# meuleman/epilogos

Hardware: AMD Instinct MI355X
Metric: Mbins scored/sec (S1, 18-state, 833 biosamples) (higher is better)
Workload: dtype u8

## Files before the change

### epilogos_amd/build.py

```python
import os
import shutil
import subprocess
from pathlib import Path

PKG = Path(__file__).resolve().parent
ROOT = PKG.parent
CSRC = PKG / "csrc"
LIB_DIR = PKG / "_lib"
LIB_PATH = LIB_DIR / "libepilogos_hip.so"
SOURCES = ["epg_abi.hip", "epg_s1.hip", "epg_s2.hip", "epg_s3.hip", "epg_s3_transpose.hip", "epg_s3_gemm.hip", "epg_s3_lanes.hip", "epg_null.hip", "epg_wide.hip", "epg_simsearch.hip",
           "epg_simsearch_prep.hip", "epg_scores_text.hip", "epg_groups.hip", "epg_null_exceed.hip", "epg_statebyline.hip", "epg_segments.hip", "epg_simsearch_pick.hip", "epg_census.hip", "epg_concordance.hip", "epg_gennorm.hip", "epg_pvals.hip", "epg_textout.hip", "epg_bgzf_inflate.hip", "epg_metrics_text.hip"]
PUBLIC_HEADERS = {"core": "epilogos_amd.h", "scores_text": "epilogos_scores_text.h", "groups": "epilogos_groups.h", "nulldraws": "epilogos_nulldraws.h",
                  "statebyline": "epilogos_statebyline.h", "segments": "epilogos_segments.h", "simsearch_pick": "epilogos_simsearch_pick.h",
                  "census": "epilogos_census.h", "concordance": "epilogos_concordance.h", "gennorm": "epilogos_gennorm.h"}
INTERNAL_HEADERS = {"pvals": "epg_pvals.h"}
WRITER_HEADERS = {"textout": "epg_textout.h"}
READER_HEADERS = {"bgzf_inflate": "epg_bgzf_inflate.h"}
METRICS_HEADERS = {"metrics_text": "epg_metrics_text.h"}
HEADERS = [CSRC / "epg_common.h", CSRC / "epg_count.h", CSRC / "epg_paircount.h", CSRC / "epg_parts.h", CSRC / "epg_pairdist.h", CSRC / "epg_text_scan.h", CSRC / "epg_text_rows.h", CSRC / "epg_fmt_f5.h", CSRC / "epg_fmt_e5.h", CSRC / "epg_bgzf_block.h", CSRC / "epg_bgzf_inflate_block.h",
           *[ROOT / "include" / name for name in PUBLIC_HEADERS.values()], *[CSRC / name for name in INTERNAL_HEADERS.values()], *[CSRC / name for name in WRITER_HEADERS.values()], *[CSRC / name for name in READER_HEADERS.values()], *[CSRC / name for name in METRICS_HEADERS.values()]]
ARCH = "gfx950"


def _hipcc():
    exe = shutil.which("hipcc") or "/opt/rocm/bin/hipcc"
    if not os.path.exists(exe):
        raise RuntimeError("hipcc not found: cannot build libepilogos_hip.so")
    return exe


def is_stale():
    if not LIB_PATH.exists():
        return True
    t = LIB_PATH.stat().st_mtime
    deps = [CSRC / s for s in SOURCES] + HEADERS
    return any(d.stat().st_mtime > t for d in deps)


IO_LIB_PATH = LIB_DIR / "libepilogos_io.so"
IO_SOURCE = CSRC / "epg_io.cpp"
IO_HEADER = ROOT / "include" / "epilogos_io.h"


def io_is_stale():
    if not IO_LIB_PATH.exists():
        return True
    t = IO_LIB_PATH.stat().st_mtime
    return any(f.stat().st_mtime > t for f in (IO_SOURCE, IO_HEADER, CSRC / "epg_deflate.h", CSRC / "epg_inflate.h", CSRC / "epg_crc32.h"))


def build_io_library(force=False, verbose=False):
    if not force and not io_is_stale():
        return IO_LIB_PATH
    LIB_DIR.mkdir(parents=True, exist_ok=True)
    cxx = shutil.which("g++") or shutil.which("c++")
    if cxx is None:
        raise RuntimeError("g++ not found: cannot build libepilogos_io.so")
    tmp = LIB_DIR / (IO_LIB_PATH.name + ".tmp.%d" % os.getpid())
    cmd = [cxx, "-O3", "-std=c++17", "-fPIC", "-shared", "-pthread", "-I" + str(ROOT / "include"), str(IO_SOURCE),
           "-lz", "-o", str(tmp)]
    if verbose:
        print(" ".join(cmd), flush=True)
    res = subprocess.run(cmd, capture_output=True, text=True)
    if res.returncode != 0:
        raise RuntimeError("g++ failed:\n" + res.stdout + res.stderr)
    os.replace(tmp, IO_LIB_PATH)
    return IO_LIB_PATH


OBJ_DIR = LIB_DIR / "obj"


def _compile_one(src, obj, extra_flags, verbose):
    cmd = [_hipcc(), "--offload-arch=" + ARCH, "-O3", "-std=c++17", "-fPIC", "-c",
           "-I" + str(ROOT / "include"), "-I" + str(CSRC), *extra_flags, str(src), "-o", str(obj)]
    if verbose:
        print(" ".join(cmd), flush=True)
    res = subprocess.run(cmd, capture_output=True, text=True)
    if res.returncode != 0:
        raise RuntimeError("hipcc failed on %s:\n%s%s" % (src.name, res.stdout, res.stderr))


def build_library(force=False, verbose=False, extra_flags=()):
    if os.environ.get("EPILOGOS_BUILD_EXPERIMENTS") == "1":
        extra_flags = tuple(extra_flags) + ("-DEPILOGOS_BUILD_EXPERIMENTS",)
    if not force and not is_stale():
        return LIB_PATH
    from concurrent.futures import ThreadPoolExecutor
    OBJ_DIR.mkdir(parents=True, exist_ok=True)
    flag_tag = OBJ_DIR / "flags.txt"
    flags_now = " ".join(extra_flags)
    same_flags = flag_tag.exists() and flag_tag.read_text() == flags_now
    hdr_t = max(h.stat().st_mtime for h in HEADERS)
    todo, objs = [], []
    for s in SOURCES:
        src, obj = CSRC / s, OBJ_DIR / (s + ".o")
        objs.append(obj)
        if force or not same_flags or not obj.exists() or obj.stat().st_mtime < max(src.stat().st_mtime, hdr_t):
            todo.append((src, obj))
    jobs = max(1, min(len(todo), int(os.environ.get("EPILOGOS_BUILD_JOBS", os.cpu_count() or 4))))
    if todo:
        with ThreadPoolExecutor(max_workers=jobs) as pool:
# ... 18 lines not shown
```

### epilogos_amd/csrc/epg_count.h

```cpp
#pragma once
#include "epg_common.h"
#include "epg_parts.h"

namespace epg {

#define EPG_B3(a, b, c, tt) ((u32)__builtin_amdgcn_bitop3_b32((int)(a), (int)(b), (int)(c), (tt)))

__device__ __forceinline__ u32 sel(u32 m, u32 x, u32 y) { return EPG_B3(m, x, y, 0xCA); }

__device__ __forceinline__ u32 dbl(u32 x) {
    u32 r;
    asm("v_add_u32 %0, %1, %1" : "=v"(r) : "v"(x));
    return r;
}

__device__ __forceinline__ void bit_planes(const u32 (&w)[8], u32 (&P)[5]) {
    const u32 n0 = sel(0x0f0f0f0fu, w[0], w[1] << 4);
    const u32 n1 = sel(0x0f0f0f0fu, w[2], w[3] << 4);
    const u32 n2 = sel(0x0f0f0f0fu, w[4], w[5] << 4);
    const u32 n3 = sel(0x0f0f0f0fu, w[6], w[7] << 4);
    const u32 m0 = sel(0x33333333u, n0, n1 << 2), m1 = sel(0x33333333u, n2, n3 << 2);
    const u32 r0 = sel(0xccccccccu, n1, n0 >> 2), r1 = sel(0xccccccccu, n3, n2 >> 2);
    P[0] = sel(0x55555555u, m0, dbl(m1)); P[1] = sel(0xaaaaaaaau, m1, m0 >> 1);
    P[2] = sel(0x55555555u, r0, dbl(r1)); P[3] = sel(0xaaaaaaaau, r1, r0 >> 1);
    const u32 c00 = sel(0x10101010u, w[0], dbl(w[4])), c01 = sel(0x10101010u, w[1], dbl(w[5]));
    const u32 c10 = sel(0x10101010u, w[2], dbl(w[6])), c11 = sel(0x10101010u, w[3], dbl(w[7]));
    const u32 d0 = sel(0x30303030u, c00, c10 << 2), d1 = sel(0x30303030u, c01, c11 << 2);
    P[4] = sel(0xf0f0f0f0u, d1, d0 >> 4);
}

__device__ __forceinline__ void low_three(const u32 (&P)[5], u32 (&L)[8]) {
    L[0] = EPG_B3(P[0], P[1], P[2], 0x01); L[1] = EPG_B3(P[0], P[1], P[2], 0x10); L[2] = EPG_B3(P[0], P[1], P[2], 0x04); L[3] = EPG_B3(P[0], P[1], P[2], 0x40);
    L[4] = EPG_B3(P[0], P[1], P[2], 0x02); L[5] = EPG_B3(P[0], P[1], P[2], 0x20); L[6] = EPG_B3(P[0], P[1], P[2], 0x08); L[7] = EPG_B3(P[0], P[1], P[2], 0x80);
}

__device__ __forceinline__ u32 indicator(const u32 (&L)[8], const u32 (&P)[5], int s) {
    switch (s >> 3) {
        case 0: return EPG_B3(L[s & 7], P[3], P[4], 0x10);
        case 1: return EPG_B3(L[s & 7], P[3], P[4], 0x40);
        case 2: return EPG_B3(L[s & 7], P[3], P[4], 0x20);
        default: return EPG_B3(L[s & 7], P[3], P[4], 0x80);
    }
}

template <int S>
__device__ __forceinline__ void count_group(const u32 (&w)[8], u32 (&cnt)[S]) {
    u32 P[5], L[8];
    bit_planes(w, P);
    low_three(P, L);
#pragma unroll
    for (int s = 0; s < S; ++s) cnt[s] += (u32)__builtin_popcount(indicator(L, P, s));
}

struct RowGeom {
    int chunks;
    int last;
    u32 tail[4];
};

__device__ __forceinline__ RowGeom make_geom(int N) {
    RowGeom g;
    g.chunks = (N + 15) >> 4;
    g.last = g.chunks - 1;
    const int t = N - 16 * g.last;
#pragma unroll
    for (int d = 0; d < 4; ++d) {
        int v = t - 4 * d;
        v = v < 0 ? 0 : (v > 4 ? 4 : v);
        g.tail[d] = v == 4 ? 0u : (0xffffffffu << (8 * v));
    }
    return g;
}

template <bool MAYBE_TAIL>
__device__ __forceinline__ void load_slot(const char* rowp, int i, int j, const RowGeom& g, u32* w) {
    const int c = 4 * i + j;
    if (!MAYBE_TAIL) {
        const uint4 v = ld16(rowp + 16 * c);
        w[0] = v.x; w[1] = v.y; w[2] = v.z; w[3] = v.w;
    } else {
        const int cc = c < g.last ? c : g.last;
        const uint4 v = ld16(rowp + 16 * cc);
        const u32 inv = c > g.last ? 0xffffffffu : 0u;
        const bool is_last = c == g.last;
// ... 20 lines not shown
}

template <int NC, typename Group>
__device__ __forceinline__ void for_each_group(const char* rowp, int j, const RowGeom& g, u32 (&cnt)[NC], Group group) {
    const int ngroups = (g.chunks + 7) >> 3;
    for (int t0 = 0; t0 < ngroups; t0 += 4) {
        u32 w[4][8];
#pragma unroll
        for (int k = 0; k < 4; ++k) {
            const int t = t0 + k;
            if (t < ngroups - 1) load_group<false>(rowp, t, j, g, w[k]);
            else if (t == ngroups - 1) load_group<true>(rowp, t, j, g, w[k]);
        }
#pragma unroll
        for (int k = 0; k < 4; ++k)
            if (t0 + k < ngroups) group(t0 + k, w[k], cnt);
    }
}

template <int S, int NG>
__device__ __forceinline__ void count_row(const char* rowp, int j, const RowGeom& g, u32 (&cnt)[S]) {
    if constexpr (NG > 0) {
        u32 w[NG][8];
        load_groups<NG>(rowp, j, g, w);
#pragma unroll
        for (int t = 0; t < NG; ++t) count_group<S>(w[t], cnt);
    } else {
        for_each_group(rowp, j, g, cnt, [](int, const u32 (&w)[8], u32 (&c)[S]) { count_group<S>(w, c); });
    }
}

template <int S, int NG>
struct CountRow {
    __device__ __forceinline__ void operator()(const char* rowp, int j, const RowGeom& g, u32 (&cnt)[S]) const { count_row<S, NG>(rowp, j, g, cnt); }
};

template <int S, typename Count, typename Epilogue, typename Finish>
__device__ __forceinline__ void super_tile(const char* __restrict__ X, long R, long ldx, const RowGeom& g, long lst, int j, int b, Count&& count,
                                           Epilogue&& epilogue, Finish&& finish) {
#pragma unroll
    for (int half = 0; half < 2; ++half) {
        const long row = lst * 32 + half * 16 + b;
        const bool valid = row < R;
        u32 cnt[S];
#pragma unroll
        for (int s = 0; s < S; ++s) cnt[s] = 0;
        count(X + (valid ? row : R - 1) * ldx, j, g, cnt);
        epilogue(half, row, valid, cnt);
    }
    const long row0 = lst * 32;
    finish(lst, row0, (int)(R - row0 < 32 ? R - row0 : 32));
}

template <int S, int NG, int NW = 4, typename Epilogue, typename Finish, typename Count = CountRow<S, NG>>
__device__ __forceinline__ void tile_loop(const char* __restrict__ X, long R, int N, long ldx, Epilogue&& epilogue, Finish&& finish,
                                          Count&& count = Count()) {
    const int lane = threadIdx.x & 63;
    const int wave = __builtin_amdgcn_readfirstlane(threadIdx.x >> 6);
    const int j = lane & 3, b = lane >> 2;
    const RowGeom g = make_geom(N);
    const long nsuper = (R + 31) >> 5;
    for (long st = (long)blockIdx.x * NW + wave; st < nsuper; st += (long)gridDim.x * NW)
        super_tile<S>(X, R, ldx, g, st, j, b, count, epilogue, finish);
}

typedef u32 epg_ldsx4 __attribute__((ext_vector_type(4)));

template <int NG>
struct DmaHalfTile {
    static constexpr int NI = 2 * NG;
    u32 soff[NI];
    u64 rpack;
    char* slot;
    u32 rd, rd_tail[2];
    int npieces;

    __device__ __forceinline__ void init(char* ring, int wave, int lane, const RowGeom& g, long ldx) {
        const int j = lane & 3, b = lane >> 2, C = g.chunks;
        npieces = 16 * C;
        slot = ring + wave * (256 * C);
        rpack = 0;
#pragma unroll
        for (int i = 0; i < NI; ++i) {
            const int p = 64 * i + lane;
            int r = p / C;
            const int c = p - r * C;
            const bool used = r < 16;
            r = used ? r : 0;
            soff[i] = used ? (u32)r * (u32)ldx + 16u * (u32)c : 0u;
            rpack |= (u64)r << (4 * i);
        }
        const u32 row = (u32)(uintptr_t)slot + 16u * (u32)(b * C);
        rd = row + 16u * j;
#pragma unroll
        for (int k = 0; k < 2; ++k) {
            const int c = 4 * (NI - 2 + k) + j;
            rd_tail[k] = row + 16u * (u32)(c < g.last ? c : g.last);
        }
    }

    __device__ __forceinline__ void fill(const char* __restrict__ X, long R, long ldx, long row0, int lane) const {
        const char* Xh = X + row0 * ldx;
        const long left = R - row0;
        auto piece = [&](int i, const char* src) {
            if (i < NI - 2 || 64 * i + lane < npieces)
                __builtin_amdgcn_global_load_lds((const __attribute__((address_space(1))) void*)src,
                                                 (__attribute__((address_space(3))) void*)(slot + 1024 * i), 16, 0, 2 );
        };
        if (left >= 16) {
#pragma unroll
            for (int i = 0; i < NI; ++i) piece(i, Xh + soff[i]);
        } else {
#pragma unroll
            for (int i = 0; i < NI; ++i) piece(i, (long)((rpack >> (4 * i)) & 15) < left ? Xh + soff[i] : X);
        }
    }

    static __device__ __forceinline__ void wait() { asm volatile("s_waitcnt vmcnt(0)" ::: "memory"); }

    __device__ __forceinline__ void read(const RowGeom& g, int j, u32 (&w)[NG][8]) const {
        epg_ldsx4 v[NI];
        __builtin_amdgcn_sched_barrier(0);
#pragma unroll
        for (int i = 0; i < NI - 2; ++i) asm volatile("ds_read_b128 %0, %1 offset:%2" : "=v"(v[i]) : "v"(rd), "n"(64 * i) : "memory");
        asm volatile("ds_read_b128 %0, %1" : "=v"(v[NI - 2]) : "v"(rd_tail[0]) : "memory");
        asm volatile("ds_read_b128 %0, %1" : "=v"(v[NI - 1]) : "v"(rd_tail[1]) : "memory");
#pragma unroll
        for (int i = 0; i < NI; ++i) asm volatile("s_waitcnt lgkmcnt(0)" : "+v"(v[i])::"memory");
        __builtin_amdgcn_sched_barrier(0);
#pragma unroll
        for (int i = 0; i < NI; ++i) {
            u32* o = &w[i >> 1][4 * (i & 1)];
            o[0] = v[i].x; o[1] = v[i].y; o[2] = v[i].z; o[3] = v[i].w;
            if (i >= NI - 2) {
                const int c = 4 * i + j;
                const u32 inv = c > g.last ? 0xffffffffu : 0u;
                const bool is_last = c == g.last;
#pragma unroll
                for (int d = 0; d < 4; ++d) o[d] |= inv | (is_last ? g.tail[d] : 0u);
            }
        }
    }
};

template <int S, int NG, int NW = 4, typename Epilogue, typename Finish>
__device__ __forceinline__ void tile_loop_dma(const char* __restrict__ X, long R, int N, long ldx, char* ring, Epilogue&& epilogue, Finish&& finish) {
    const int lane = threadIdx.x & 63;
    const int wave = __builtin_amdgcn_readfirstlane(threadIdx.x >> 6);
    const int j = lane & 3, b = lane >> 2;
    const RowGeom g = make_geom(N);
    const long nsuper = (R + 31) >> 5, stride = (long)gridDim.x * NW;
    long st = (long)blockIdx.x * NW + wave;
    if (st >= nsuper) return;
    DmaHalfTile<NG> dma;
    dma.init(ring, wave, lane, g, ldx);
    dma.fill(X, R, ldx, st * 32, lane);
    dma.wait();
    for (; st < nsuper; st += stride) {
#pragma unroll
        for (int half = 0; half < 2; ++half) {
            const long row = st * 32 + half * 16 + b;
            u32 w[NG][8];
            dma.read(g, j, w);
            if (half == 0) dma.fill(X, R, ldx, st * 32 + 16, lane);
            else if (st + stride < nsuper) dma.fill(X, R, ldx, (st + stride) * 32, lane);
            u32 cnt[S];
#pragma unroll
            for (int s = 0; s < S; ++s) cnt[s] = 0;
#pragma unroll
            for (int t = 0; t < NG; ++t) count_group<S>(w[t], cnt);
            dma.wait();
            epilogue(half, row, row < R, cnt);
        }
        const long row0 = st * 32;
        finish(st, row0, (int)(R - row0 < 32 ? R - row0 : 32));
    }
}

constexpr int KH_MAXP = 48;
struct KhParts {
    const char* x[KH_MAXP];
    u16* h[KH_MAXP];
    long rows[KH_MAXP];
    long ldx[KH_MAXP];
    long t0[KH_MAXP + 1];
    int n_cols[KH_MAXP];
    int n;
};

template <int S, int NG, int NW = 4, typename Enter, typename Epilogue, typename Finish>
__device__ __forceinline__ void tile_loop_parts(const KhParts& pt, Enter&& enter, Epilogue&& epilogue, Finish&& finish) {
    const int lane = threadIdx.x & 63;
    const int wave = __builtin_amdgcn_readfirstlane(threadIdx.x >> 6);
    const int j = lane & 3, b = lane >> 2;
    const long nsuper = pt.t0[pt.n];
    PartCursor at;
    int part = -1;
    const char* X = nullptr;
    long R = 0, ldx = 0, base = 0;
    RowGeom g = make_geom(16);
    for (long st = (long)blockIdx.x * NW + wave; st < nsuper; st += (long)gridDim.x * NW) {
        at.advance(pt.t0, st, 32);
        if (at.part != part) {
            part = at.part;
            X = pt.x[part];
            R = pt.rows[part];
            ldx = pt.ldx[part];
            base = pt.t0[part];
            g = make_geom(pt.n_cols[part]);
            enter(part);
        }
        super_tile<S>(X, R, ldx, g, st - base, j, b, CountRow<S, NG>(), epilogue, finish);
    }
}

template <int S>
__device__ __forceinline__ void pack_reduce(const u32 (&cnt)[S], u32 (&d)[(S + 1) / 2]) {
#pragma unroll
    for (int m = 0; m < (S + 1) / 2; ++m) {
        const u32 hi = 2 * m + 1 < S ? cnt[2 * m + 1] : 0u;
        d[m] = quad_sum(cnt[2 * m] | (hi << 16));
    }
}

__device__ __forceinline__ u32 sel4(u32 x0, u32 x1, u32 x2, u32 x3, int j) {
    const u32 lo = (j & 1) ? x1 : x0;
    const u32 hi = (j & 1) ? x3 : x2;
    return (j & 2) ? hi : lo;
}

template <int ND>
__device__ __forceinline__ u32 quad_state_count(const u32 (&d)[ND], int k, int j) {
    const u32 lo = d[2 * k], hi = 2 * k + 1 < ND ? d[2 * k + 1] : 0u;
    const u32 v = (j & 2) ? hi : lo;
    return (j & 1) ? v >> 16 : v & 0xffffu;
}

template <int S, bool WHOLE_DWORDS>
__device__ __forceinline__ void stage_hist_row(char* srow, const u32 (&d)[(S + 1) / 2], int j, int Sout) {
    constexpr int ND = (S + 1) / 2;
    if constexpr (WHOLE_DWORDS) {
        static_assert((S & 1) == 0, "whole dwords need an even row");
#pragma unroll
        for (int k = 0; k < (ND + 3) / 4; ++k) {
            const u32 v = sel4(d[4 * k], 4 * k + 1 < ND ? d[4 * k + 1] : 0u, 4 * k + 2 < ND ? d[4 * k + 2] : 0u, 4 * k + 3 < ND ? d[4 * k + 3] : 0u, j);
            if (4 * k + j < ND) *reinterpret_cast<u32*>(srow + 4 * (4 * k + j)) = v;
        }
    } else {
#pragma unroll
        for (int k = 0; k < (S + 3) / 4; ++k) {
            const u32 c = quad_state_count(d, k, j);
            if (4 * k + j < Sout) *reinterpret_cast<u16*>(srow + 2 * (4 * k + j)) = (u16)c;
        }
    }
}

template <int S>
struct StateTotals {
    static constexpr int ND = (S + 1) / 2;
    u32 accp[ND];
    int since, flush_every;
    __device__ __forceinline__ void init(int nmax) {
#pragma unroll
        for (int m = 0; m < ND; ++m) accp[m] = 0;
        flush_every = 65535 / nmax > 1 ? 65535 / nmax - 1 : 1;
        since = 0;
    }
    __device__ __forceinline__ void flush(u64* s_cnt, int j) {
        if (j == 0) {
#pragma unroll
            for (int m = 0; m < ND; ++m) {
                const u32 lo = accp[m] & 0xffffu, hi = accp[m] >> 16;
                if (lo) atomicAdd(&s_cnt[2 * m], (u64)lo);
                if (hi) atomicAdd(&s_cnt[2 * m + 1], (u64)hi);
            }
        }
#pragma unroll
        for (int m = 0; m < ND; ++m) accp[m] = 0;
        since = 0;
    }
    __device__ __forceinline__ void add(const u32 (&d)[ND], bool valid, u64* s_cnt, int j) {
#pragma unroll
        for (int m = 0; m < ND; ++m) accp[m] += valid ? d[m] : 0u;
        if (++since >= flush_every) flush(s_cnt, j);
    }
    __device__ __forceinline__ void commit(u64* s_cnt, int j, u64* __restrict__ counts, int Sout) {
        flush(s_cnt, j);
        __syncthreads();
        if ((int)threadIdx.x < Sout && s_cnt[threadIdx.x]) atomicAdd(&counts[threadIdx.x], s_cnt[threadIdx.x]);
    }
};

}
```

### epilogos_amd/csrc/epg_s1.hip

```cpp
#include "epg_count.h"
#include "epg_paircount.h"

#include <stdlib.h>
#include <string.h>

namespace epg {

constexpr int K1P_LD = 17;

template <int SC, bool FULL, bool PAIRS, typename Loop>
__device__ __forceinline__ void bin_hist_body(int Sout_, u64* __restrict__ counts, int nmax, u64* __restrict__ counts2, Loop&& loop) {
    constexpr int S = SC;
    constexpr int ND = (S + 1) / 2;
    const int Sout = FULL ? S : Sout_;
    const int ROWB = 2 * Sout;
    __shared__ u64 s_cnt[S + 1];
    __shared__ __attribute__((aligned(16))) char s_stage[4][32 * 2 * S];
    constexpr int PG = (S + 2) / 3, PSP = 3 * PG, PROLES = PG * (PG + 1) / 2, PSLICE = PROLES <= 64 ? 64 / PROLES : 1;
    static_assert(!PAIRS || (FULL && PROLES <= 64), "the pair counts need a compile-time row width and at most 64 block roles");
    __shared__ u32 s_pair[PAIRS ? 4 * PSP * K1P_LD : 1];
    __shared__ u64 s_c2[PAIRS ? S * S : 1];
    const int lane = threadIdx.x & 63, wave = threadIdx.x >> 6;
    const int j = lane & 3, b = lane >> 2;
    if (threadIdx.x <= S) s_cnt[threadIdx.x] = 0;
    if (PAIRS) {
        for (int e = threadIdx.x; e < S * S; e += 256) s_c2[e] = 0;
        for (int e = threadIdx.x; e < 4 * PSP * K1P_LD; e += 256) s_pair[e] = 0;
    }
    __syncthreads();
    u16* H = nullptr;
    int pgi = -1, pgj = 0, pkq = 0;
    u64 pacc[PAIRS ? 9 : 1], prs[PAIRS ? 3 : 1];
    if (PAIRS) {
        const int role = lane < PROLES * PSLICE ? lane / PSLICE : -1;
        pkq = lane % PSLICE;
        if (role >= 0) pair_role(role, PG, pgi, pgj);
#pragma unroll
        for (int c = 0; c < 9; ++c) pacc[c] = 0;
#pragma unroll
        for (int c = 0; c < 3; ++c) prs[c] = 0;
    }
    auto pair_counts = [&](const char* stage, int rows) {
        u32* sp = s_pair + wave * PSP * K1P_LD;
        const u16* raw = reinterpret_cast<const u16*>(stage);
        __builtin_amdgcn_wave_barrier();
        for (int e = lane; e < S * 16; e += 64) {
            const int i = e >> 4, k = e & 15;
            const u32 lo = 2 * k < rows ? raw[(2 * k) * S + i] : 0u, hi = 2 * k + 1 < rows ? raw[(2 * k + 1) * S + i] : 0u;
            sp[i * K1P_LD + k] = lo | (hi << 16);
        }
        __builtin_amdgcn_wave_barrier();
        if (pgi >= 0) {
            u32 part[9], ps[3];
            pair_tile_dot(sp + 3 * pgi * K1P_LD, sp + 3 * pgj * K1P_LD, K1P_LD, pkq, 16, PSLICE, pgi == pgj, part, ps);
#pragma unroll
            for (int c = 0; c < 9; ++c) pacc[c] += part[c];
#pragma unroll
            for (int c = 0; c < 3; ++c) prs[c] += ps[c];
        }
        __builtin_amdgcn_wave_barrier();
    };

    StateTotals<S> totals;
    totals.init(nmax);

    auto enter = [&](u16* Hpart) { H = Hpart; };
    auto epilogue = [&](int half, long row, bool valid, u32 (&cnt)[S]) {
        u32 d[ND];
        pack_reduce<S>(cnt, d);
        if (counts) totals.add(d, valid, s_cnt, j);
        if (H) stage_hist_row<S, FULL && (S & 1) == 0>(&s_stage[wave][(half * 16 + b) * ROWB], d, j, Sout);
    };
    auto finish = [&](long st, long row0, int rows) {
        if (H) store_staged(s_stage[wave], reinterpret_cast<char*>(H) + row0 * ROWB, rows * ROWB, lane);
        if constexpr (PAIRS) pair_counts(s_stage[wave], rows);
    };
    loop(enter, epilogue, finish);

    if (counts) totals.commit(s_cnt, j, counts, Sout);
    if constexpr (PAIRS) {
        if (pgi >= 0) pair_fold(pacc, prs, pgi, pgj, S, s_c2);
        pair_commit(s_c2, S, counts2);
    }
}

template <int SC, int NG, bool FULL, bool DMA = false>
__global__ __launch_bounds__(256) void k_bin_hist(const char* __restrict__ X, long R, int N, long ldx, int Sout_,
                                                   u16* __restrict__ H, u64* __restrict__ counts) {
    extern __shared__ __attribute__((aligned(16))) char s_ring[];
    bin_hist_body<SC, FULL, false>(Sout_, counts, N, nullptr, [&](auto&& enter, auto&& epilogue, auto&& finish) {
        enter(H);
        if constexpr (DMA) tile_loop_dma<SC, NG>(X, R, N, ldx, s_ring, epilogue, finish);
        else tile_loop<SC, NG>(X, R, N, ldx, epilogue, finish);
    });
}

template <int SC, int NG>
__global__ __launch_bounds__(256) void k_bin_hist_s2(const char* __restrict__ X, long R, int N, long ldx, u16* __restrict__ H,
                                                      u64* __restrict__ counts, u64* __restrict__ counts2) {
    bin_hist_body<SC, true, true>(SC, counts, N, counts2, [&](auto&& enter, auto&& epilogue, auto&& finish) {
        enter(H);
        tile_loop<SC, NG>(X, R, N, ldx, epilogue, finish);
    });
}

template <int SC, int NG, bool FULL>
__global__ __launch_bounds__(256) void k_bin_hist_parts(const KhParts pt, int Sout_, u64* __restrict__ counts, int nmax) {
    bin_hist_body<SC, FULL, false>(Sout_, counts, nmax, nullptr, [&](auto&& enter, auto&& epilogue, auto&& finish) {
        tile_loop_parts<SC, NG>(pt, [&](int part) { enter(pt.h[part]); }, epilogue, finish);
    });
}

__global__ __launch_bounds__(256) void k_bin_hist_safe(const char* __restrict__ X, long row_begin, long row_end, int N,
                                                        long ldx, int S, u16* __restrict__ H, u64* __restrict__ counts, int mask = 31) {
    __shared__ u32 s_h[4][128];
    const int lane = threadIdx.x & 63, wave = threadIdx.x >> 6;
    for (long row = row_begin + (long)blockIdx.x * 4 + wave; row < row_end; row += (long)gridDim.x * 4) {
        for (int s = lane; s < S; s += 64) s_h[wave][s] = 0;
        __builtin_amdgcn_wave_barrier();
        const char* rp = X + row * ldx;
        for (int n = lane; n < N; n += 64) {
            const int v = (unsigned char)rp[n] & mask;
            if (v < S) atomicAdd(&s_h[wave][v], 1u);
        }
        __builtin_amdgcn_wave_barrier();
        for (int s = lane; s < S; s += 64) {
            const u32 c = s_h[wave][s];
            if (H) H[row * S + s] = (u16)c;
            if (counts && c) atomicAdd(&counts[s], (u64)c);
        }
        __builtin_amdgcn_wave_barrier();
    }
}

__global__ void k_s1_table(const float* __restrict__ q, int N, int S, double* __restrict__ T64, float* __restrict__ T32) {
    const long e = (long)blockIdx.x * blockDim.x + threadIdx.x;
    if (e >= (long)(N + 1) * S) return;
    const int c = (int)(e / S), s = (int)(e % S);
    const double p = (double)c / (double)N;
    const double v = kl_term(p, (double)q[s]);
    T64[e] = v;
    T32[e] = (float)v;
}

template <int S, int NG, typename OT>
__global__ __launch_bounds__(256) void k_score_s1(const char* __restrict__ X, long R, int N, long ldx,
                                                   const OT* __restrict__ T, OT* __restrict__ out) {
    constexpr int ND = (S + 1) / 2;
    constexpr int ROWB = S * (int)sizeof(OT);
    __shared__ __attribute__((aligned(16))) char s_stage[4][32 * ROWB];
    const int lane = threadIdx.x & 63, wave = threadIdx.x >> 6;
    const int j = lane & 3, b = lane >> 2;
    auto epilogue = [&](int half, long row, bool valid, u32 (&cnt)[S]) {
        u32 d[ND];
        pack_reduce<S>(cnt, d);
        OT* srow = reinterpret_cast<OT*>(&s_stage[wave][(half * 16 + b) * ROWB]);
#pragma unroll
        for (int k = 0; k < (S + 3) / 4; ++k) {
            const u32 c = quad_state_count(d, k, j);
            const int s = 4 * k + j;
            if (s < S) srow[s] = (c && valid) ? T[(long)c * S + s] : (OT)0;
        }
    };
    auto finish = [&](long st, long row0, int rows) {
        store_staged_nt(s_stage[wave], reinterpret_cast<char*>(out) + row0 * ROWB, rows * ROWB, lane);
    };
    tile_loop<S, NG>(X, R, N, ldx, epilogue, finish);
}

template <typename OT, bool LDS_T>
__global__ __launch_bounds__(LDS_T ? 1024 : 256) void k_score_s1_from_hist(const u16* __restrict__ H, long total, int S,
                                                                             const OT* __restrict__ Tg, int nent, OT* __restrict__ out,
                                                                             u64* __restrict__ zero_counts, int rev) {
    extern __shared__ __attribute__((aligned(16))) char smem_t[];
    if (zero_counts && blockIdx.x == 0 && (int)threadIdx.x < S) zero_counts[threadIdx.x] = 0;
    const OT* T = Tg;
    if (LDS_T) {
        OT* Ts = reinterpret_cast<OT*>(smem_t);
        for (int e = threadIdx.x; e < nent; e += blockDim.x) Ts[e] = Tg[e];
        __syncthreads();
        T = Ts;
    }
    const u32 cmax = (u32)(nent / S - 1);
    const long nquads = total >> 2;
    const long stride = (long)gridDim.x * blockDim.x;
    long qd = (long)blockIdx.x * blockDim.x + threadIdx.x;
    const long qtop = nquads - 1, qsgn = rev ? -1 : 1, qoff = rev ? qtop : 0;
    for (; qd + 3 * stride < nquads; qd += 4 * stride) {
        uint2 h[4];
#pragma unroll
        for (int u = 0; u < 4; ++u) h[u] = *reinterpret_cast<const uint2*>(H + 4 * (qoff + qsgn * (qd + u * stride)));
#pragma unroll
// ... 47 lines not shown
        const long long t = s_part[0] + s_part[1] + s_part[2] + s_part[3];
        if (t) atomicAdd(reinterpret_cast<u64*>(total), (u64)t);
    }
}

template <typename IT>
__global__ __launch_bounds__(256) void k_normalise(const IT* __restrict__ C, long n, const long long* __restrict__ total,
                                                    float* __restrict__ q) {
    const double tot = (double)(*total);
    for (long i = (long)blockIdx.x * blockDim.x + threadIdx.x; i < n; i += (long)gridDim.x * blockDim.x)
        q[i] = (float)((double)C[i] / tot);
}

template <typename IT>
__global__ __launch_bounds__(256) void k_normalise_small(const IT* __restrict__ C, int n, float* __restrict__ q) {
    __shared__ long long s_part[4];
    long long acc = 0;
    for (int i = threadIdx.x; i < n; i += 256) acc += (long long)C[i];
    for (int off = 32; off > 0; off >>= 1) acc += __shfl_down(acc, off);
    if ((threadIdx.x & 63) == 0) s_part[threadIdx.x >> 6] = acc;
    __syncthreads();
    const double tot = (double)(s_part[0] + s_part[1] + s_part[2] + s_part[3]);
    for (int i = threadIdx.x; i < n; i += 256) q[i] = (float)((double)C[i] / tot);
}

static int blocks_per_cu() { return g_force[FORCE_K1_BLOCKS_PER_CU] > 0 ? g_force[FORCE_K1_BLOCKS_PER_CU] : 2; }
int grid_for_tiles(long R) {
    const long nsuper = (R + 31) >> 5;
    long blocks = (nsuper + 3) / 4;
    const long cap = (long)num_cus() * blocks_per_cu();
    if (blocks > cap) {
        const long iters = (nsuper + cap * 4 - 1) / (cap * 4);
        blocks = (nsuper + iters * 4 - 1) / (iters * 4);
    }
    if (blocks < 1) blocks = 1;
    return (int)blocks;
}

template <typename F>
static void with_count_core(int S, int ng, F&& f) {
    if (S == 15 || S == 18 || S == 25)
        with_constant<25, 15, 18>(S, [&](auto sc) {
            with_constant<0, 1, 2, 3, 4, 5, 6, 7, 8>(ng, [&](auto NG) { f(sc, NG, std::true_type{}); });
        });
    else
        with_constant<31, 15, 18, 25>(S < 15 ? 15 : S < 18 ? 18 : S < 25 ? 25 : 31,
                                      [&](auto sc) { f(sc, std::integral_constant<int, 0>{}, std::false_type{}); });
}

static bool dma_rows_ok(const char* X, long ldx) {
    return !g_force[FORCE_K1_PLAIN_LOADS] && ((reinterpret_cast<uintptr_t>(X) | (uintptr_t)ldx) & 15) == 0 && ldx < (1L << 27);
}

long fast_rows(long R, int N, long ldx) {
    const long chunks = (N + 15) / 16;
    const long over = 16 * chunks - ldx;
    if (over <= 0) return R;
    const long unsafe = (over + ldx - 1) / ldx;
    return R > unsafe ? R - unsafe : 0;
}

extern "C" int epg_bin_hist(const int8_t* X8, int64_t R, int32_t N, int64_t ldx, int32_t S, uint16_t* H, int64_t* counts, void* stream) {
    hipStream_t st = (hipStream_t)stream;
    if (R < 0 || N < 1 || ldx < N || S < 1) return fail(EPG_ERR_INVALID_ARG, "bin_hist: bad shape R=%lld N=%d ldx=%lld S=%d", (long long)R, N, (long long)ldx, S);
    if (S > 127) return fail(EPG_ERR_UNSUPPORTED, "bin_hist: S=%d > 127 (states are int8)", S);
    if (N > 65535) return fail(EPG_ERR_UNSUPPORTED, "bin_hist: N=%d > 65535 (uint16 per-bin counts)", N);
    if (R == 0) return EPG_OK;
    if (!X8) return fail(EPG_ERR_INVALID_ARG, "bin_hist: X is NULL");
    if (H && (reinterpret_cast<uintptr_t>(H) & 15)) return fail(EPG_ERR_INVALID_ARG, "bin_hist: H must be 16-byte aligned");
    const char* X = reinterpret_cast<const char*>(X8);
    u64* cnt = reinterpret_cast<u64*>(counts);
    if (S > 31) {
        hipLaunchKernelGGL(k_bin_hist_safe, dim3((unsigned)((R + 3) / 4 < num_cus() * 32L ? (R + 3) / 4 : num_cus() * 32L)), dim3(256), 0, st, X, 0L,
                           (long)R, N, ldx, S, H, cnt, 255);
        EPG_LAUNCH_CHECK("k_bin_hist_safe");
        return EPG_OK;
    }
    const long Rf = fast_rows(R, N, ldx);
    if (Rf > 0) {
        hipError_t dyn = hipSuccess;
        with_count_core(S, (N + 127) / 128, [&](auto SC, auto NG, auto MODEL) {
            constexpr bool FULL = MODEL && (SC & 1) == 0;
            if constexpr (MODEL && NG > 0) {
                if (dma_rows_ok(X, ldx)) {
                    static DynLds lds;
                    const int ring = 1024 * ((N + 15) / 16);
                    dyn = ensure_dyn_lds(lds, reinterpret_cast<const void*>(k_bin_hist<SC, NG, FULL, true>), 1024 * 8 * NG);
                    if (dyn == hipSuccess)
                        hipLaunchKernelGGL((k_bin_hist<SC, NG, FULL, true>), dim3(grid_for_tiles(Rf)), dim3(256), ring, st, X, Rf, N, ldx, S, H, cnt);
                    return;
                }
            }
            hipLaunchKernelGGL((k_bin_hist<SC, NG, FULL>), dim3(grid_for_tiles(Rf)), dim3(256), 0, st, X, Rf, N, ldx, S, H, cnt);
        });
        if (dyn != hipSuccess) return fail(EPG_ERR_HIP, "bin_hist: the LDS ring was refused: %s", hipGetErrorString(dyn));
        EPG_LAUNCH_CHECK("k_bin_hist");
    }
    if (Rf < R) {
        hipLaunchKernelGGL(k_bin_hist_safe, dim3((unsigned)((R - Rf + 3) / 4 < 1024 ? (R - Rf + 3) / 4 : 1024)), dim3(256), 0, st, X, Rf, (long)R, N, ldx, S, H, cnt);
        EPG_LAUNCH_CHECK("k_bin_hist_safe");
    }
    return EPG_OK;
}

extern "C" int epg_bin_hist_s2(const int8_t* X8, int64_t R, int32_t N, int64_t ldx, int32_t S, uint16_t* H, int64_t* counts, int64_t* counts2,
                               void* stream) {
    hipStream_t st = (hipStream_t)stream;
    if (!H || !counts2) return fail(EPG_ERR_INVALID_ARG, "bin_hist_s2: H and counts2 are required");
    const bool fused = (S == 15 || S == 18 || S == 25) && R > 0 && N >= 1 && N <= 1024 && ldx >= N && X8 &&
                       !(reinterpret_cast<uintptr_t>(H) & 15) && fast_rows(R, N, ldx) == R;
    if (!fused) {
        int rc = epg_bin_hist(X8, R, N, ldx, S, H, counts, stream);
        if (rc) return rc;
        return epg_hist_s2_from_binhist(H, R, S, counts2, stream);
    }
    const char* X = reinterpret_cast<const char*>(X8);
    u64* c1 = reinterpret_cast<u64*>(counts);
    u64* c2 = reinterpret_cast<u64*>(counts2);
    with_constant<25, 18, 15>(S, [&](auto SC) {
        with_constant<8, 1, 2, 3, 4, 5, 6, 7>((N + 127) / 128, [&](auto NG) {
            hipLaunchKernelGGL((k_bin_hist_s2<decltype(SC)::value, NG>), dim3(grid_for_tiles(R)), dim3(256), 0, st, X, R, N, ldx, H, c1, c2);
        });
    });
    EPG_LAUNCH_CHECK("k_bin_hist_s2");
    return EPG_OK;
}

extern "C" int epg_bin_hist_parts(int32_t nparts, const int8_t* const* X, const int64_t* R, const int32_t* N, const int64_t* ldx, int32_t S,
                                  uint16_t* const* H, int64_t* counts, void* stream) {
    hipStream_t st = (hipStream_t)stream;
    if (nparts < 0 || (nparts && (!X || !R || !N || !ldx))) return fail(EPG_ERR_INVALID_ARG, "bin_hist_parts: NULL argument array");
    if (S < 1 || S > 127) return fail(EPG_ERR_UNSUPPORTED, "bin_hist_parts: S=%d outside 1..127", S);
    for (int p = 0; p < nparts; ++p) {
        if (R[p] < 0 || (R[p] && (N[p] < 1 || ldx[p] < N[p]))) return fail(EPG_ERR_INVALID_ARG, "bin_hist_parts: bad shape of part %d", p);
        if (R[p] && N[p] > 65535) return fail(EPG_ERR_UNSUPPORTED, "bin_hist_parts: N=%d > 65535 (uint16 per-bin counts)", N[p]);
        if (R[p] && !X[p]) return fail(EPG_ERR_INVALID_ARG, "bin_hist_parts: X of part %d is NULL", p);
        if (H && H[p] && (reinterpret_cast<uintptr_t>(H[p]) & 15)) return fail(EPG_ERR_INVALID_ARG, "bin_hist_parts: H of part %d must be 16-byte aligned", p);
    }
    if (S > 31) {
        for (int p = 0; p < nparts; ++p) {
            const int rc = epg_bin_hist(X[p], R[p], N[p], ldx[p], S, H ? H[p] : nullptr, counts, stream);
            if (rc) return rc;
        }
        return EPG_OK;
    }
    u64* cnt = reinterpret_cast<u64*>(counts);
    for (int p = 0; p < nparts; ++p) {
        const long Rf = R[p] ? fast_rows(R[p], N[p], ldx[p]) : 0;
        if (Rf == R[p]) continue;
        hipLaunchKernelGGL(k_bin_hist_safe, dim3((unsigned)((R[p] - Rf + 3) / 4 < 1024 ? (R[p] - Rf + 3) / 4 : 1024)), dim3(256), 0, st,
                           reinterpret_cast<const char*>(X[p]), Rf, (long)R[p], N[p], (long)ldx[p], S, H ? H[p] : nullptr, cnt);
        EPG_LAUNCH_CHECK("k_bin_hist_safe");
    }
    auto cls = [](int n) { const int ng = (n + 127) / 128; return ng <= 8 ? ng : 0; };
    for (int c = 0; c <= 8; ++c) {
        for (int p0 = 0; p0 < nparts;) {
            KhParts pt;
            int nmax = 1;
            p0 = pack_parts(pt, p0, nparts, 32, [&](int p) { return R[p] && cls(N[p]) == c ? fast_rows(R[p], N[p], ldx[p]) : 0L; },
                            [&](int k, int p) {
                                pt.x[k] = reinterpret_cast<const char*>(X[p]); pt.h[k] = H ? H[p] : nullptr;
                                pt.ldx[k] = ldx[p]; pt.n_cols[k] = N[p];
                                if (N[p] > nmax) nmax = N[p];
                            });
            if (pt.n == 0) break;
            with_count_core(S, c, [&](auto SC, auto NG, auto) {
                hipLaunchKernelGGL((k_bin_hist_parts<SC, NG, (NG > 0 && (SC & 1) == 0)>), dim3(grid_for_tiles(pt.t0[pt.n] * 32)), dim3(256), 0, st, pt, S,
                                   cnt, nmax);
            });
            EPG_LAUNCH_CHECK("k_bin_hist_parts");
        }
    }
    return EPG_OK;
}

static int64_t s1_table_bytes(int N, int S) { return align_up((int64_t)(N + 1) * S * 8, 256) + align_up((int64_t)(N + 1) * S * 4, 256); }

int64_t s1_ws_bytes(int64_t R, int N, int S) {
    return s1_table_bytes(N, S) + 256 + align_up(R * S * 2, 256);
}

static int build_s1_table(const float* q, int N, int S, void* ws, double** T64, float** T32, hipStream_t st) {
    *T64 = reinterpret_cast<double*>(ws);
    *T32 = reinterpret_cast<float*>(reinterpret_cast<char*>(ws) + align_up((int64_t)(N + 1) * S * 8, 256));
    const long n = (long)(N + 1) * S;
    hipLaunchKernelGGL(k_s1_table, dim3((int)((n + 255) / 256)), dim3(256), 0, st, q, N, S, *T64, *T32);
    EPG_LAUNCH_CHECK("k_s1_table");
    return EPG_OK;
}
static int check_score_from_hist_args(const uint16_t* H, const double* out64, const float* out32) {
    if ((reinterpret_cast<uintptr_t>(H) & 7) != 0) return fail(EPG_ERR_INVALID_ARG, "score_s1_from_binhist: H must be 8-byte aligned");
    if ((out32 && (reinterpret_cast<uintptr_t>(out32) & 15)) || (out64 && (reinterpret_cast<uintptr_t>(out64) & 15)))
        return fail(EPG_ERR_INVALID_ARG, "score_s1_from_binhist: outputs must be 16-byte aligned");
    return EPG_OK;
}

template <typename OT>
static int launch_score_s1_from_hist_t(const uint16_t* H, long total, int32_t S, const OT* T, int nent, OT* out, u64* zero_counts, hipStream_t st) {
    const size_t tbytes = (size_t)nent * sizeof(OT);
    const int rev = 1;
    if (tbytes <= 150 * 1024) {
        const int per_cu = tbytes <= 75 * 1024 ? 2 : 1;
        long nb = (total / 4 + 4095) / 4096;
        if (nb > (long)num_cus() * per_cu) nb = (long)num_cus() * per_cu;
        if (nb < 1) nb = 1;
        auto kern = k_score_s1_from_hist<OT, true>;
        static DynLds lds_attr;
        EPG_HIP(ensure_dyn_lds(lds_attr, reinterpret_cast<const void*>(kern), 150 * 1024));
        hipLaunchKernelGGL(kern, dim3((int)nb), dim3(1024), tbytes, st, H, total, S, T, nent, out, zero_counts, rev);
    } else {
        long nb = (total / 4 + 1023) / 1024;
        if (nb > num_cus() * 8L) nb = num_cus() * 8L;
        if (nb < 1) nb = 1;
        hipLaunchKernelGGL((k_score_s1_from_hist<OT, false>), dim3((int)nb), dim3(256), 0, st, H, total, S, T, nent, out, zero_counts, rev);
    }
    EPG_LAUNCH_CHECK("k_score_s1_from_hist");
    return EPG_OK;
}

static int launch_score_s1_from_hist(const uint16_t* H, int64_t R, int32_t N, int32_t S, const double* T64, const float* T32,
                                     double* out64, float* out32, hipStream_t st, u64* zero_counts = nullptr) {
    const long total = (long)R * S;
    const int nent = (N + 1) * S;
    int rc = EPG_OK;
    if (out32) rc = launch_score_s1_from_hist_t<float>(H, total, S, T32, nent, out32, zero_counts, st);
    if (!rc && out64) rc = launch_score_s1_from_hist_t<double>(H, total, S, T64, nent, out64, out32 ? nullptr : zero_counts, st);
    return rc;
}


extern "C" int epg_score_s1_from_binhist(const uint16_t* H, int64_t R, int32_t N, int32_t S, const float* q, double* out64, float* out32,
                                         void* ws, int64_t ws_bytes, void* stream) {
    hipStream_t st = (hipStream_t)stream;
    if (R < 0 || N < 1 || S < 1) return fail(EPG_ERR_INVALID_ARG, "score_s1: bad shape");
    if (R == 0) return EPG_OK;
    if (!H || !q || !ws) return fail(EPG_ERR_INVALID_ARG, "score_s1_from_binhist: NULL argument");
    if (ws_bytes < s1_table_bytes(N, S)) return fail(EPG_ERR_WORKSPACE, "score_s1: workspace %lld < %lld bytes", (long long)ws_bytes, (long long)s1_table_bytes(N, S));
    int rc = check_score_from_hist_args(H, out64, out32);
    if (rc) return rc;
    double* T64; float* T32;
    rc = build_s1_table(q, N, S, ws, &T64, &T32, st);
    if (rc) return rc;
    return launch_score_s1_from_hist(H, R, N, S, T64, T32, out64, out32, st);
}

extern "C" int epg_score_s1_from_binhist_table(const uint16_t* H, int64_t R, int32_t N, int32_t S, const double* T64, const float* T32,
                                               double* out64, float* out32, void* stream) {
    if (R < 0 || N < 1 || S < 1) return fail(EPG_ERR_INVALID_ARG, "score_s1: bad shape");
    if (R == 0) return EPG_OK;
    if (!H || (out64 && !T64) || (out32 && !T32)) return fail(EPG_ERR_INVALID_ARG, "score_s1_from_binhist_table: NULL argument");
    if ((T64 && (reinterpret_cast<uintptr_t>(T64) & 7)) || (T32 && (reinterpret_cast<uintptr_t>(T32) & 3)))
        return fail(EPG_ERR_INVALID_ARG, "score_s1_from_binhist_table: misaligned table");
// ... 114 lines not shown
```

Measured before the change: 6066.

## Extend LDS DMA ring loading to pair-count and multi-part histogram kernels

```diff
diff --git a/epilogos_amd/build.py b/epilogos_amd/build.py
--- a/epilogos_amd/build.py
+++ b/epilogos_amd/build.py
@@ -17,7 +17,7 @@
 WRITER_HEADERS = {"textout": "epg_textout.h"}
 READER_HEADERS = {"bgzf_inflate": "epg_bgzf_inflate.h"}
 METRICS_HEADERS = {"metrics_text": "epg_metrics_text.h"}
-HEADERS = [CSRC / "epg_common.h", CSRC / "epg_count.h", CSRC / "epg_paircount.h", CSRC / "epg_parts.h", CSRC / "epg_pairdist.h", CSRC / "epg_text_scan.h", CSRC / "epg_text_rows.h", CSRC / "epg_fmt_f5.h", CSRC / "epg_fmt_e5.h", CSRC / "epg_bgzf_block.h", CSRC / "epg_bgzf_inflate_block.h",
+HEADERS = [CSRC / "epg_common.h", CSRC / "epg_count.h", CSRC / "epg_paircount.h", CSRC / "epg_parts.h", CSRC / "epg_dma_rows.h", CSRC / "epg_pairdist.h", CSRC / "epg_text_scan.h", CSRC / "epg_text_rows.h", CSRC / "epg_fmt_f5.h", CSRC / "epg_fmt_e5.h", CSRC / "epg_bgzf_block.h", CSRC / "epg_bgzf_inflate_block.h",
            *[ROOT / "include" / name for name in PUBLIC_HEADERS.values()], *[CSRC / name for name in INTERNAL_HEADERS.values()], *[CSRC / name for name in WRITER_HEADERS.values()], *[CSRC / name for name in READER_HEADERS.values()], *[CSRC / name for name in METRICS_HEADERS.values()]]
 ARCH = "gfx950"
 
diff --git a/epilogos_amd/csrc/epg_count.h b/epilogos_amd/csrc/epg_count.h
--- a/epilogos_amd/csrc/epg_count.h
+++ b/epilogos_amd/csrc/epg_count.h
@@ -1,5 +1,6 @@
 #pragma once
 #include "epg_common.h"
+#include "epg_dma_rows.h"
 #include "epg_parts.h"
 
 namespace epg {
@@ -186,15 +187,10 @@
         rpack = 0;
 #pragma unroll
         for (int i = 0; i < NI; ++i) {
-            const int p = 64 * i + lane;
-            int r = p / C;
-            const int c = p - r * C;
-            const bool used = r < 16;
-            r = used ? r : 0;
-            soff[i] = used ? (u32)r * (u32)ldx + 16u * (u32)c : 0u;
+            const int r = dma_piece_row(i, lane, C, ldx, &soff[i]);
             rpack |= (u64)r << (4 * i);
         }
-        const u32 row = (u32)(uintptr_t)slot + 16u * (u32)(b * C);
+        const u32 row = (u32)(uintptr_t)slot + dma_slot_chunk(b, 0, C);
         rd = row + 16u * j;
 #pragma unroll
         for (int k = 0; k < 2; ++k) {
@@ -204,10 +200,11 @@
     }
 
     __device__ __forceinline__ void fill(const char* __restrict__ X, long R, long ldx, long row0, int lane) const {
-        const char* Xh = X + row0 * ldx;
+        const long base = row0 * ldx;
+        const char* Xh = X + base;
         const long left = R - row0;
         auto piece = [&](int i, const char* src) {
-            if (i < NI - 2 || 64 * i + lane < npieces)
+            if (dma_piece_issued(i, lane, NI, npieces))
                 __builtin_amdgcn_global_load_lds((const __attribute__((address_space(1))) void*)src,
                                                  (__attribute__((address_space(3))) void*)(slot + 1024 * i), 16, 0, 2 );
         };
@@ -216,7 +213,7 @@
             for (int i = 0; i < NI; ++i) piece(i, Xh + soff[i]);
         } else {
 #pragma unroll
-            for (int i = 0; i < NI; ++i) piece(i, (long)((rpack >> (4 * i)) & 15) < left ? Xh + soff[i] : X);
+            for (int i = 0; i < NI; ++i) piece(i, X + dma_piece_src(base, soff[i], (int)((rpack >> (4 * i)) & 15), left));
         }
     }
 
@@ -247,37 +244,56 @@
     }
 };
 
-template <int S, int NG, int NW = 4, typename Epilogue, typename Finish>
-__device__ __forceinline__ void tile_loop_dma(const char* __restrict__ X, long R, int N, long ldx, char* ring, Epilogue&& epilogue, Finish&& finish) {
+struct DmaTile {
+    const char* X;
+    long R, lst;
+};
+
+struct OneMatrixTiles {
+    const char* X;
+    long R;
+    __device__ __forceinline__ DmaTile counting(long st) { return {X, R, st}; }
+    __device__ __forceinline__ DmaTile asking(long st) { return {X, R, st}; }
+};
+
+template <int S, int NG, int NW = 4, typename Tiles, typename Epilogue, typename Finish>
+__device__ __forceinline__ void tile_loop_dma(Tiles&& tiles, long nsuper, int N, long ldx, char* ring, Epilogue&& epilogue, Finish&& finish) {
     const int lane = threadIdx.x & 63;
     const int wave = __builtin_amdgcn_readfirstlane(threadIdx.x >> 6);
     const int j = lane & 3, b = lane >> 2;
     const RowGeom g = make_geom(N);
-    const long nsuper = (R + 31) >> 5, stride = (long)gridDim.x * NW;
+    const long stride = (long)gridDim.x * NW;
     long st = (long)blockIdx.x * NW + wave;
     if (st >= nsuper) return;
     DmaHalfTile<NG> dma;
     dma.init(ring, wave, lane, g, ldx);
-    dma.fill(X, R, ldx, st * 32, lane);
+    {
+        const DmaTile first = tiles.asking(st);
+        dma.fill(first.X, first.R, ldx, first.lst * 32, lane);
+    }
     dma.wait();
     for (; st < nsuper; st += stride) {
+        const DmaTile t = tiles.counting(st);
 #pragma unroll
         for (int half = 0; half < 2; ++half) {
-            const long row = st * 32 + half * 16 + b;
+            const long row = t.lst * 32 + half * 16 + b;
             u32 w[NG][8];
             dma.read(g, j, w);
-            if (half == 0) dma.fill(X, R, ldx, st * 32 + 16, lane);
-            else if (st + stride < nsuper) dma.fill(X, R, ldx, (st + stride) * 32, lane);
+            if (half == 0) dma.fill(t.X, t.R, ldx, t.lst * 32 + 16, lane);
+            else if (st + stride < nsuper) {
+                const DmaTile nx = tiles.asking(st + stride);
+                dma.fill(nx.X, nx.R, ldx, nx.lst * 32, lane);
+            }
             u32 cnt[S];
 #pragma unroll
             for (int s = 0; s < S; ++s) cnt[s] = 0;
 #pragma unroll
-            for (int t = 0; t < NG; ++t) count_group<S>(w[t], cnt);
+            for (int t2 = 0; t2 < NG; ++t2) count_group<S>(w[t2], cnt);
             dma.wait();
-            epilogue(half, row, row < R, cnt);
-        }
-        const long row0 = st * 32;
-        finish(st, row0, (int)(R - row0 < 32 ? R - row0 : 32));
+            epilogue(half, row, row < t.R, cnt);
+        }
+        const long row0 = t.lst * 32;
+        finish(t.lst, row0, (int)(t.R - row0 < 32 ? t.R - row0 : 32));
     }
 }
 
@@ -318,6 +334,33 @@
     }
 }
 
+template <typename Enter>
+struct PartTiles {
+    const KhParts& pt;
+    Enter enter;
+    PartsAhead at;
+    int part = -1;
+    const char* X = nullptr;
+    long R = 0, base = 0;
+    __device__ __forceinline__ DmaTile counting(long st) {
+        at.counting(pt.t0, st);
+        const int p = __builtin_amdgcn_readfirstlane(at.cur.part);
+        if (p != part) {
+            part = p;
+            X = pt.x[p];
+            R = pt.rows[p];
+            base = pt.t0[p];
+            enter(p);
+        }
+        return {X, R, st - base};
+    }
+    __device__ __forceinline__ DmaTile asking(long st) {
+        at.asking(pt.t0, st);
+        const int p = __builtin_amdgcn_readfirstlane(at.pre.part);
+        return {pt.x[p], pt.rows[p], st - pt.t0[p]};
+    }
+};
+
 template <int S>
 __device__ __forceinline__ void pack_reduce(const u32 (&cnt)[S], u32 (&d)[(S + 1) / 2]) {
 #pragma unroll
diff --git a/epilogos_amd/csrc/epg_dma_rows.h b/epilogos_amd/csrc/epg_dma_rows.h
--- /dev/null
+++ b/epilogos_amd/csrc/epg_dma_rows.h
@@ -0,0 +1,38 @@
+#pragma once
+#include "epg_parts.h"
+
+namespace epg {
+
+EPG_HOST_DEVICE int dma_piece_row(int i, int lane, int C, long ldx, uint32_t* soff) {
+    const int p = 64 * i + lane;
+    int r = p / C;
+    const int c = p - r * C;
+    const bool used = r < 16;
+    r = used ? r : 0;
+    *soff = used ? (uint32_t)r * (uint32_t)ldx + 16u * (uint32_t)c : 0u;
+    return r;
+}
+
+EPG_HOST_DEVICE bool dma_piece_issued(int i, int lane, int NI, int npieces) { return i < NI - 2 || 64 * i + lane < npieces; }
+
+EPG_HOST_DEVICE long dma_piece_src(long base, uint32_t soff, int r, long left) { return (long)r < left ? base + (long)soff : 0L; }
+
+EPG_HOST_DEVICE uint32_t dma_piece_dst(int i, int lane) { return 1024u * (uint32_t)i + 16u * (uint32_t)lane; }
+EPG_HOST_DEVICE uint32_t dma_slot_chunk(int b, int c, int C) { return 16u * (uint32_t)(b * C + c); }
+
+struct PartsAhead {
+    PartCursor cur, pre;
+    EPG_HOST_DEVICE long counting(const long* t0, long st) { return cur.advance(t0, st, 32); }
+    EPG_HOST_DEVICE long asking(const long* t0, long st) { return pre.advance(t0, st, 32); }
+};
+
+template <typename Parts>
+static bool dma_parts_ok(const Parts& pt) {
+    for (int k = 0; k < pt.n; ++k)
+        if (pt.n_cols[k] != pt.n_cols[0] || pt.ldx[k] != pt.ldx[0] || ((reinterpret_cast<uintptr_t>(pt.x[k]) | (uintptr_t)pt.ldx[k]) & 15) != 0 ||
+            pt.ldx[k] >= (1L << 27))
+            return false;
+    return pt.n > 0;
+}
+
+}
diff --git a/epilogos_amd/csrc/epg_s1.hip b/epilogos_amd/csrc/epg_s1.hip
--- a/epilogos_amd/csrc/epg_s1.hip
+++ b/epilogos_amd/csrc/epg_s1.hip
@@ -7,6 +7,11 @@
 namespace epg {
 
 constexpr int K1P_LD = 17;
+
+constexpr int bin_hist_static_lds(int S, bool pairs) {
+    return 8 * (S + 1) + 4 * 32 * 2 * S + (pairs ? 4 * 3 * ((S + 2) / 3) * K1P_LD * 4 + 8 * S * S : 4 + 8) + 64;
+}
+constexpr bool dma_ring_fits(int S, int NG, bool pairs) { return bin_hist_static_lds(S, pairs) + 1024 * 8 * NG <= 80 * 1024; }
 
 template <int SC, bool FULL, bool PAIRS, typename Loop>
 __device__ __forceinline__ void bin_hist_body(int Sout_, u64* __restrict__ counts, int nmax, u64* __restrict__ counts2, Loop&& loop) {
@@ -20,6 +25,7 @@
     static_assert(!PAIRS || (FULL && PROLES <= 64), "the pair counts need a compile-time row width and at most 64 block roles");
     __shared__ u32 s_pair[PAIRS ? 4 * PSP * K1P_LD : 1];
     __shared__ u64 s_c2[PAIRS ? S * S : 1];
+    static_assert(sizeof(s_cnt) + sizeof(s_stage) + sizeof(s_pair) + sizeof(s_c2) + 64 <= bin_hist_static_lds(S, PAIRS), "dma_ring_fits counts on this bound");
     const int lane = threadIdx.x & 63, wave = threadIdx.x >> 6;
     const int j = lane & 3, b = lane >> 2;
     if (threadIdx.x <= S) s_cnt[threadIdx.x] = 0;
@@ -90,24 +96,30 @@
     extern __shared__ __attribute__((aligned(16))) char s_ring[];
     bin_hist_body<SC, FULL, false>(Sout_, counts, N, nullptr, [&](auto&& enter, auto&& epilogue, auto&& finish) {
         enter(H);
-        if constexpr (DMA) tile_loop_dma<SC, NG>(X, R, N, ldx, s_ring, epilogue, finish);
+        if constexpr (DMA) tile_loop_dma<SC, NG>(OneMatrixTiles{X, R}, (R + 31) >> 5, N, ldx, s_ring, epilogue, finish);
         else tile_loop<SC, NG>(X, R, N, ldx, epilogue, finish);
     });
 }
 
-template <int SC, int NG>
+template <int SC, int NG, bool DMA = false>
 __global__ __launch_bounds__(256) void k_bin_hist_s2(const char* __restrict__ X, long R, int N, long ldx, u16* __restrict__ H,
                                                       u64* __restrict__ counts, u64* __restrict__ counts2) {
+    extern __shared__ __attribute__((aligned(16))) char s_ring[];
     bin_hist_body<SC, true, true>(SC, counts, N, counts2, [&](auto&& enter, auto&& epilogue, auto&& finish) {
         enter(H);
-        tile_loop<SC, NG>(X, R, N, ldx, epilogue, finish);
+        if constexpr (DMA) tile_loop_dma<SC, NG>(OneMatrixTiles{X, R}, (R + 31) >> 5, N, ldx, s_ring, epilogue, finish);
+        else tile_loop<SC, NG>(X, R, N, ldx, epilogue, finish);
     });
 }
 
-template <int SC, int NG, bool FULL>
+template <int SC, int NG, bool FULL, bool DMA = false>
 __global__ __launch_bounds__(256) void k_bin_hist_parts(const KhParts pt, int Sout_, u64* __restrict__ counts, int nmax) {
+    extern __shared__ __attribute__((aligned(16))) char s_ring[];
     bin_hist_body<SC, FULL, false>(Sout_, counts, nmax, nullptr, [&](auto&& enter, auto&& epilogue, auto&& finish) {
-        tile_loop_parts<SC, NG>(pt, [&](int part) { enter(pt.h[part]); }, epilogue, finish);
+        auto enter_part = [&](int part) { enter(pt.h[part]); };
+        if constexpr (DMA)
+            tile_loop_dma<SC, NG>(PartTiles<decltype(enter_part)>{pt, enter_part}, pt.t0[pt.n], pt.n_cols[0], pt.ldx[0], s_ring, epilogue, finish);
+        else tile_loop_parts<SC, NG>(pt, enter_part, epilogue, finish);
     });
 }
 
@@ -321,6 +333,7 @@
         with_count_core(S, (N + 127) / 128, [&](auto SC, auto NG, auto MODEL) {
             constexpr bool FULL = MODEL && (SC & 1) == 0;
             if constexpr (MODEL && NG > 0) {
+                static_assert(dma_ring_fits(SC, NG, false), "two workgroups per CU");
                 if (dma_rows_ok(X, ldx)) {
                     static DynLds lds;
                     const int ring = 1024 * ((N + 15) / 16);
@@ -356,11 +369,23 @@
     const char* X = reinterpret_cast<const char*>(X8);
     u64* c1 = reinterpret_cast<u64*>(counts);
     u64* c2 = reinterpret_cast<u64*>(counts2);
+    hipError_t dyn = hipSuccess;
     with_constant<25, 18, 15>(S, [&](auto SC) {
         with_constant<8, 1, 2, 3, 4, 5, 6, 7>((N + 127) / 128, [&](auto NG) {
-            hipLaunchKernelGGL((k_bin_hist_s2<decltype(SC)::value, NG>), dim3(grid_for_tiles(R)), dim3(256), 0, st, X, R, N, ldx, H, c1, c2);
+            constexpr int sc = decltype(SC)::value;
+            if constexpr (dma_ring_fits(sc, NG, true)) {
+                if (dma_rows_ok(X, ldx)) {
+                    static DynLds lds;
+                    dyn = ensure_dyn_lds(lds, reinterpret_cast<const void*>(k_bin_hist_s2<sc, NG, true>), 1024 * 8 * NG);
+                    if (dyn == hipSuccess)
+                        hipLaunchKernelGGL((k_bin_hist_s2<sc, NG, true>), dim3(grid_for_tiles(R)), dim3(256), 1024 * ((N + 15) / 16), st, X, R, N, ldx, H, c1, c2);
+                    return;
+                }
+            }
+            hipLaunchKernelGGL((k_bin_hist_s2<sc, NG>), dim3(grid_for_tiles(R)), dim3(256), 0, st, X, R, N, ldx, H, c1, c2);
         });
     });
+    if (dyn != hipSuccess) return fail(EPG_ERR_HIP, "bin_hist_s2: the LDS ring was refused: %s", hipGetErrorString(dyn));
     EPG_LAUNCH_CHECK("k_bin_hist_s2");
     return EPG_OK;
 }
@@ -403,10 +428,23 @@
                                 if (N[p] > nmax) nmax = N[p];
                             });
             if (pt.n == 0) break;
-            with_count_core(S, c, [&](auto SC, auto NG, auto) {
-                hipLaunchKernelGGL((k_bin_hist_parts<SC, NG, (NG > 0 && (SC & 1) == 0)>), dim3(grid_for_tiles(pt.t0[pt.n] * 32)), dim3(256), 0, st, pt, S,
-                                   cnt, nmax);
+            hipError_t dyn = hipSuccess;
+            with_count_core(S, c, [&](auto SC, auto NG, auto MODEL) {
+                constexpr bool FULL = NG > 0 && (SC & 1) == 0;
+                const dim3 grid(grid_for_tiles(pt.t0[pt.n] * 32));
+                if constexpr (MODEL && NG > 0) {
+                    static_assert(dma_ring_fits(SC, NG, false), "two workgroups per CU");
+                    if (!g_force[FORCE_K1_PLAIN_LOADS] && dma_parts_ok(pt)) {
+                        static DynLds lds;
+                        dyn = ensure_dyn_lds(lds, reinterpret_cast<const void*>(k_bin_hist_parts<SC, NG, FULL, true>), 1024 * 8 * NG);
+                        if (dyn == hipSuccess)
+                            hipLaunchKernelGGL((k_bin_hist_parts<SC, NG, FULL, true>), grid, dim3(256), 1024 * ((pt.n_cols[0] + 15) / 16), st, pt, S, cnt, nmax);
+                        return;
+                    }
+                }
+                hipLaunchKernelGGL((k_bin_hist_parts<SC, NG, FULL>), grid, dim3(256), 0, st, pt, S, cnt, nmax);
             });
+            if (dyn != hipSuccess) return fail(EPG_ERR_HIP, "bin_hist_parts: the LDS ring was refused: %s", hipGetErrorString(dyn));
             EPG_LAUNCH_CHECK("k_bin_hist_parts");
         }
     }
```

Result: slower. 5812 (-4.2%).
